# Frank-Wang-oss/GNN_RUL_Benchmarking

Measured on AMD Instinct MI355X. Metric: training samples/sec, C-MAPSS FD004-shaped ST_GCN, higher is better.
Workload: dtype f32 (f16x2-split MFMA operands, fp32 accumulate); 1 GPU; ST_GCN.update (fwd+MSE+bwd+Adam), C-MAPSS FD004-shaped windows [14 sensors x 30], per-GPU batch 65536, dropout 0.2, lr 0.0001, wd 0.0001; per_gpu_batch=65536, global_batch=65536, num_patch=14, patch_size=30, parallelism=dp1, batchnorm=single process, loss_readback=end of run (device-side loss each step)

## Files before the change

### gnn_rul_benchmarking_amd/csrc/stgcn_train_layout.hpp

```cpp
#pragma once
#include "stgcn_device.hpp"
#include "stgcn_host.hpp"

namespace rulgnn {

struct StepScratch {
    uint32_t drop_key[8];
    float lr_over_bc1, inv_sqrt_bc2;
    double bn_count;
    uint32_t pad[4];
};
static_assert(sizeof(StepScratch) == 64, "step scratch layout");
constexpr uint32_t WS_CLEAN_TOKEN = 0x52554C43u;

struct HeadScalars {
    StepScratch* sc;
    uint64_t seed, step;
    int L, has_adam;
    int64_t adam_step;
    float lr, beta1, beta2;
    double bn_count;
};
__device__ __forceinline__ void head_scalars(const HeadScalars& h, int tid) {
    StepScratch* sc = h.sc;
    if (tid == 0) {
        sc->bn_count = h.bn_count;
        if (sc->pad[1] != WS_CLEAN_TOKEN) {
            sc->pad[0] = 2u;
            sc->pad[2] = 0u;
        }
        sc->pad[1] = 0u;
    }
    if (tid >= 64 && tid < 72) sc->drop_key[tid - 64] = tid - 64 < h.L ? dropout_layer_key(h.seed, h.step, tid - 64) : 0u;
    if (h.has_adam && tid == 128) {
        const double bc1 = 1.0 - pow((double)h.beta1, (double)h.adam_step);
        const double bc2 = 1.0 - pow((double)h.beta2, (double)h.adam_step);
        sc->lr_over_bc1 = (float)((double)h.lr / bc1);
        sc->inv_sqrt_bc2 = (float)(1.0 / sqrt(bc2));
    }
}

constexpr int CELL_REPLICAS = 16;
__host__ __device__ constexpr int cell_fwd(int L) { (void)L; return 0; }
__host__ __device__ constexpr int cell_bwd(int L) { return 2 * L * 2 * F; }
__host__ __device__ constexpr int cell_loss(int L) { return 2 * (2 * L * 2 * F); }
__host__ __device__ constexpr int cell_stride(int L) { return 2 * (2 * L * 2 * F) + 8; }
__host__ __device__ __forceinline__ StepScratch* step_scratch(double* cells, int L) {
    return reinterpret_cast<StepScratch*>(cells + CELL_REPLICAS * cell_stride(L));
}
__host__ __device__ __forceinline__ unsigned* step_barrier(double* cells, int L) {
    return reinterpret_cast<unsigned*>(reinterpret_cast<char*>(step_scratch(cells, L)) + sizeof(StepScratch));
}
__device__ __forceinline__ double cell_sum(const double* cells, int L, int i) {
    double v = 0.0;
#pragma unroll
    for (int r = 0; r < CELL_REPLICAS; ++r) v += cells[r * cell_stride(L) + i];
    return v;
}

constexpr int BN_TABLE_ROWS = 7;
template <bool COHERENT = false>
__device__ __forceinline__ void bn_pair_to_lds(const double* cells, const float* prm, float* bnc, int L, int N, bool fwd, int b, int lane) {
    const int CS = cell_stride(L);
    const int base = (fwd ? cell_fwd(L) : cell_bwd(L)) + b * 2 * F;
    double v = 0.0;
    if (lane < 2 * F) {
        if constexpr (COHERENT) {
            double t[CELL_REPLICAS];
#pragma unroll
            for (int r = 0; r < CELL_REPLICAS; ++r) t[r] = __hip_atomic_load(&cells[r * CS + base + lane], __ATOMIC_RELAXED, __HIP_MEMORY_SCOPE_AGENT);
#pragma unroll
            for (int r = 0; r < CELL_REPLICAS; ++r) v += t[r];
        } else {
#pragma unroll
        for (int r = 0; r < CELL_REPLICAS; ++r) v += cells[r * CS + base + lane];
        }
    }
    const double s1 = v, s2 = __shfl(v, (lane + F) & 63, 64);
    if (lane < F) {
        const int c = lane;
        const double cnt = step_scratch(const_cast<double*>(cells), L)->bn_count;
        float* o = bnc + b * BN_TABLE_ROWS * F;
        if (fwd) {
            const double mean = s1 / cnt;
            double var = s2 / cnt - mean * mean;
            var = var < 0.0 ? 0.0 : var;
            const double istd = 1.0 / sqrt(var + (double)BN_EPS);
            const int LS = layer_stride(N);
            const double g = prm[(b / 2) * LS + off_bn_g(N, b % 2) + c];
            o[0 * F + c] = (float)mean;
            o[1 * F + c] = (float)istd;
            o[2 * F + c] = (float)g;
            o[3 * F + c] = prm[(b / 2) * LS + off_bn_b(N, b % 2) + c];
            o[4 * F + c] = (float)(g * istd);
        } else {
            o[5 * F + c] = (float)(s1 / cnt);
            o[6 * F + c] = (float)(s2 / cnt);
        }
    }
}

}
```

### gnn_rul_benchmarking_amd/csrc/stgcn_train_mx.hip

```cpp
#include <algorithm>
#include <cstdlib>
#include <type_traits>

#include "stgcn_host.hpp"
#include "stgcn_mx.hpp"
#include "stgcn_train_layout.hpp"
#include "stgcn_train_mx.hpp"
#include "stgcn_train_mx_ops.hpp"

namespace rulgnn {

#ifdef MXP_TRACE
__device__ unsigned mxp_ts[128];
__device__ int mxp_n;
__device__ unsigned mxp_id[128];
#define MXP_MARKI(ID) do { if (PERSIST && blockIdx.x == 0 && threadIdx.x == 0 && mxp_n < 128) { mxp_id[mxp_n] = ID; mxp_ts[mxp_n++] = (unsigned)wall_clock64(); } } while (0)
#define MXP_MARK() MXP_MARKI(0)
#else
#define MXP_MARK() do {} while (0)
#define MXP_MARKI(ID) do {} while (0)
#endif
template <int L, int KIND, int IDX, int NFIX, bool PERSIST>
__device__ __forceinline__ void mxt_phase_body(const MxTrainK& a, float* smem_all, unsigned target) {
    MXP_MARKI(100 + KIND * 10 + IDX);
    const int N = NFIX ? NFIX : a.N;
    const int LS = layer_stride(N);
    const int lane = threadIdx.x & 63, wave = threadIdx.x >> 6;
    const int g = lane >> 4, col = lane & 15;
    constexpr int NBN = 2 * L;
    constexpr int CS = cell_stride(L);
    constexpr int LY = KIND == PH_TOP ? L - 1 : IDX / 2;
    constexpr int BLK = KIND == PH_TOP ? 1 : IDX % 2;
    constexpr bool WITH_PREV = KIND == PH_F && BLK == 0 && LY >= 1;
    constexpr bool BWD_PREV = KIND == PH_G && BLK == 0 && LY >= 1;
    constexpr int LIN = WITH_PREV ? LY - 1 : LY;
    constexpr bool GRAD_IN = KIND == PH_G && (BLK == 1 || LY >= 1);
    constexpr bool GRAD_TOP = GRAD_IN && LY == L - 1;
    constexpr bool NEED_SB = KIND == PH_G && BLK == 0;
    static_assert(!(KIND == PH_F && IDX == 0), "F_0 is stgcn_train_f0_mx_kernel");

    const int XF = 40 * N;
    constexpr int AF = 220;
    constexpr int SH_BNC = (NBN * MXT_BNC * F + 3) & ~3;
    float* const bnc = smem_all;
    float* const red = smem_all + SH_BNC;
    double* const pairbuf = reinterpret_cast<double*>(red + MXT_RED_FLOATS);
    const int off_zero = 0;
    const int off_scr = off_zero + MXT_ZERO_FLOATS;
    const int off_sh = off_scr + MXT_SCRATCH_FLOATS;
    const int off_X = off_sh + MXT_SHIFT_FLOATS;
    const int off_A = off_X + XF;
    const int off_SB = off_A + AF;
    const int off_DX = off_SB + (NEED_SB ? XF : 0);
    const int off_XP = off_DX + (GRAD_IN ? XF : 0);
    const int wave_floats = off_XP + (BWD_PREV ? XF : 0);
    float* const smem = smem_all + SH_BNC + MXT_RED_FLOATS + 2 * MXT_WAVES * (2 * F + 2) + wave * wave_floats;
    u32x2* const sh_tile = reinterpret_cast<u32x2*>(smem + off_sh);

    int64_t tile = (int64_t)blockIdx.x * MXT_WAVES + wave;
    const int64_t tstride = (int64_t)gridDim.x * MXT_WAVES;

    auto dma = [&](const float* src, int off, int bytes) {
        if constexpr (NFIX != 0) {
            if (bytes == 160 * NFIX) { dma_tile_fixed<160 * NFIX>(src, smem + off, lane); return; }
            if (bytes == 32 * NFIX) { dma_tile_fixed<32 * NFIX>(src, smem + off, lane); return; }
        }
        if (bytes == 4 * AF) { dma_tile_fixed<4 * AF>(src, smem + off, lane); return; }
        dma_tile(src, smem + off, bytes, lane);
    };
    auto req_XA = [&](int64_t t) {
        dma(a.xrec[LIN] + t * XF, off_X, 4 * XF);
        dma(a.arec + t * AF, off_A, 4 * AF);
    };
    auto req_SB = [&](int64_t t) { if constexpr (NEED_SB) dma(a.sb + t * XF, off_SB, 4 * XF); };
    auto req_DX = [&](int64_t t) {
        if constexpr (GRAD_TOP) dma(a.dtop + t * (8 * N), off_DX, 32 * N);
        else if constexpr (GRAD_IN) dma(a.dx + t * XF, off_DX, 4 * XF);
    };
    auto req_XP = [&](int64_t t) { if constexpr (BWD_PREV) dma(a.qrec[LY] + t * XF, off_XP, 4 * XF); };
    if (tile < a.ntiles) { req_XA(tile); req_SB(tile); req_DX(tile); req_XP(tile); }

    for (int i = lane; i < MXT_ZERO_FLOATS; i += 64) smem[off_zero + i] = 0.f;
    if (lane < 2) sh_tile[64 + 65 * lane] = u32x2{0u, 0u};
    constexpr int M0_LY = (KIND == PH_F && BLK == 0) ? 1 : 2;
    constexpr int M1_LY = (KIND == PH_F && BLK == 0) ? 0 : ((KIND == PH_F) ? 1 : ((KIND == PH_G && BLK == 0) ? 0 : 2));
    MXP_MARKI(1);
    LayerRaw rc, rp;
    layer_raw(rc, a.prm, LY, N, g, col, M0_LY, M1_LY);
    if constexpr (WITH_PREV) layer_raw(rp, a.prm, LY - 1, N, g, col, 2, 2);
    ConvOp wT = ConvOp{u32x4{0u, 0u, 0u, 0u}, u32x4{0u, 0u, 0u, 0u}};
    ThetaOp thN = ThetaOp{u32x4{0u, 0u, 0u, 0u}, u32x4{0u, 0u, 0u, 0u}};
    u32x4 ident = u32x4{0u, 0u, 0u, 0u};
    ConvRaw wT_raw = ConvRaw{{0.f, 0.f, 0.f, 0.f}, {0.f, 0.f, 0.f, 0.f}};
    ThetaRaw thN_raw = ThetaRaw{{0.f, 0.f, 0.f, 0.f}};
    if constexpr (KIND == PH_G) {
        wT_raw = conv_bwd_raw(a.prm + LY * LS + off_conv_w(N, BLK), g, col);
        if constexpr (BLK == 0 && LY >= 1) thN_raw = theta_n_raw(a.prm + LY * LS, N, g, col);
        unsigned w[4];
#pragma unroll
        for (int r = 0; r < 4; ++r) w[r] = (4 * g + r == col) ? 0x3C00u : 0u;
        const unsigned p01 = w[0] | (w[1] << 16), p23 = w[2] | (w[3] << 16);
        ident = u32x4{p01, p23, p01, p23};
    }
    {
        constexpr int FW0 = WITH_PREV ? 2 * LY - 2 : 2 * LY;
        constexpr int NFW = (KIND == PH_F && BLK == 1) || (KIND == PH_G && BLK == 0) ? 1 : 2;
        static_assert(NFW + (KIND == PH_G ? 1 : 0) <= MXT_WAVES, "one reduction pair per wavefront");
        MXP_MARKI(2);
        if constexpr (PERSIST) {
            if (threadIdx.x == 0) {
                unsigned* const ctr = step_barrier(a.cells, L);
                unsigned spins = 0;
                while (__hip_atomic_load(ctr, __ATOMIC_RELAXED, __HIP_MEMORY_SCOPE_AGENT) < target) {
                    __builtin_amdgcn_s_sleep(1);
                    if (++spins > (1u << 22)) { atomicOr(&step_scratch(a.cells, L)->pad[0], 4u); break; }
                }
            }
            __syncthreads();
        }
        constexpr bool COH = PERSIST;
        MXP_MARKI(3);
        if (wave < NFW) bn_pair_to_lds<COH>(a.cells, a.prm, bnc, L, N, true, FW0 + wave, lane);
        if (KIND == PH_G && wave == NFW) bn_pair_to_lds<COH>(a.cells, a.prm, bnc, L, N, false, IDX, lane);
        if constexpr (KIND == PH_G) {
            wT = conv_bwd_pack(wT_raw);
            if constexpr (BLK == 0 && LY >= 1) thN = theta_pack(thN_raw);
        }
        __syncthreads();
    }
    MXP_MARKI(4);
    LayerK kc;
    layer_constants(kc, rc, bnc, LY, g, col, M0_LY, M1_LY);
    LayerK kp;
    if constexpr (WITH_PREV) layer_constants(kp, rp, bnc, LY - 1, g, col, 2, 2);
    float bA[3] = {0.f, 0.f, 0.f}, bk1[3] = {0.f, 0.f, 0.f}, bk2[3] = {0.f, 0.f, 0.f};
    if constexpr (KIND == PH_G) {
        const float* q = bnc + IDX * MXT_BNC * F;
#pragma unroll
        for (int r = 0; r < 3; ++r) {
            const int c = slot_chan(4 * g + r);
            bA[r] = c >= 0 ? q[4 * F + c] : 0.f;
            bk1[r] = c >= 0 ? q[5 * F + c] * a.gscale : 0.f;
            bk2[r] = c >= 0 ? q[6 * F + c] * a.gscale : 0.f;
        }
    }
    float fc1w[16], fc1wT[16];
    float fc1b = 0.f, fc2w = 0.f, fc2b = 0.f;
    if constexpr (KIND == PH_TOP) {
        const int colc = col < N ? col : 0;
#pragma unroll
        for (int k = 0; k < 16; ++k) {
            const int kc2 = k < N ? k : 0;
            const float v = a.prm[off_fc1_w(N, L) + colc * N + kc2], vt = a.prm[off_fc1_w(N, L) + kc2 * N + colc];
            fc1w[k] = (col < N && k < N) ? v : 0.f;
            fc1wT[k] = (col < N && k < N) ? vt : 0.f;
        }
        const float b1 = a.prm[off_fc1_b(N, L) + colc], w2 = a.prm[off_fc2_w(N, L) + colc];
        fc1b = col < N ? b1 : 0.f;
        fc2w = col < N ? w2 : 0.f;
        fc2b = a.prm[off_fc2_b(N, L)];
    }

    const bool col_ok = col < N;
    const float colm = col_ok ? 1.f : 0.f;
    const int pitch = 4 * N;
    int xoff[3], aoff[3], chan[3];
#pragma unroll
    for (int r = 0; r < 3; ++r) {
        const int c = slot_chan(4 * g + r);
        chan[r] = c;
        xoff[r] = (c >= 0 && col_ok) ? c * pitch + col : -1;
    }
    {
        const int cc = slot_chan(col);
#pragma unroll
        for (int r = 0; r < 3; ++r) {
            const int c = slot_chan(4 * g + r);
            aoff[r] = (c >= 0 && cc >= 0) ? sym(c, cc) : -1;
        }
    }
    auto ld_tile = [&](int base, float (&v)[4][3]) {
#pragma unroll
        for (int s = 0; s < 4; ++s)
#pragma unroll
            for (int r = 0; r < 3; ++r) v[s][r] = smem[(xoff[r] >= 0 ? base + xoff[r] : off_zero) + s * N];
    };
    auto st_tile = [&](float* dst, const float (&v)[4][3], int ns) {
#pragma unroll
        for (int s = 0; s < 4; ++s)
            if (s < ns) {
#pragma unroll
                for (int r = 0; r < 3; ++r)
                    if (xoff[r] >= 0) dst[xoff[r] + s * N] = v[s][r];
            }
    };
    const int sh_rd1 = col >= 1 ? lane - 1 : 64, sh_rd2 = col >= 2 ? lane - 2 : 64;
    int sh_rd1_lo = sh_rd1 + 65, sh_rd2_lo = sh_rd2 + 65;
    const int sh_bk = col + (BLK == 0 ? 1 : 2) < 16 ? lane + (BLK == 0 ? 1 : 2) : 64;
    int sh_bk_lo = sh_bk + 65;
    asm volatile("" : "+v"(sh_rd1_lo), "+v"(sh_rd2_lo), "+v"(sh_bk_lo));
    const unsigned t_bias = g == 3 ? 0x3C00u << 16 : 0u;
    uint32_t dkey[L];
#pragma unroll
    for (int l = 0; l < L; ++l) dkey[l] = step_scratch(a.cells, L)->drop_key[l];
    uint32_t dro[3];
#pragma unroll
    for (int r = 0; r < 3; ++r) dro[r] = (uint32_t)((chan[r] >= 0 ? chan[r] : 0) * N + col);
    const bool use_drop = a.dropout_p > 0.f;

    float s_a[3] = {0.f, 0.f, 0.f}, s_b[3] = {0.f, 0.f, 0.f};
    f32x4 acc_w0 = {0.f, 0.f, 0.f, 0.f}, acc_w1 = {0.f, 0.f, 0.f, 0.f};
    f32x4 acc_th = {0.f, 0.f, 0.f, 0.f};
    float acc_b = 0.f, acc_w2 = 0.f, acc_b2 = 0.f, acc_loss = 0.f;
    const float inv_gb = 1.0f / (float)a.global_batch;

    auto stage_T = [&](const auto& X, const auto& adjB, auto& T, auto& xo) {
        constexpr int NS = std::extent_v<std::remove_reference_t<decltype(T)>>;
#pragma unroll
        for (int s = 0; s < NS; ++s) {
            const Split2 p01 = split2(X[s][0], X[s][1]), p2 = split2(X[s][2], 0.f);
            const Op2 o = {u32x4{p01.hi, p2.hi, p01.hi, p2.hi}, u32x4{p01.lo, p2.lo, p01.lo, p2.lo}};
            xo[s] = o;
            T[s] = mfma16z(o.h, adjB[s]);
            T[s] = mfma16(o.l, adjB[s], T[s]);
        }
        __builtin_amdgcn_sched_barrier(0);
    };
    auto stage_Hp = [&](const auto& T, const ThetaOp& th, auto& Hp) {
        constexpr int NS = std::extent_v<std::remove_reference_t<decltype(Hp)>>;
#pragma unroll
        for (int s = 0; s < NS; ++s) {
            const Split2 p01 = split2(T[s][0], T[s][1]), p23 = split2(T[s][2], T[s][3]);
            const u32x4 ta = {p01.hi, p23.hi | t_bias, p01.lo, p23.lo};
            Hp[s] = mfma16z(ta, th.hi);
            Hp[s] = mfma16(ta, th.lo, Hp[s]);
        }
        __builtin_amdgcn_sched_barrier(0);
    };
    auto stage_conv = [&](const auto& D, float partner, const ConvOp& w, int rd, int rd_lo, auto& z, auto& keep, auto& keep_sh) {
        constexpr int NS = std::extent_v<std::remove_reference_t<decltype(z)>>;
        u32x4 bh[NS], bl[NS];
#pragma unroll
        for (int s = 0; s < NS; ++s) {
            const Pk p = pack3(D[s][0], D[s][1], D[s][2], partner);
            const Shifted prev = shift_read(sh_tile, rd, rd_lo, lane, p);
            bh[s] = cat(p.hi, prev.hi);
            bl[s] = cat(p.lo, prev.lo);
            keep[s] = p;
            keep_sh[s] = prev;
            __builtin_amdgcn_sched_barrier(0);
        }
        __builtin_amdgcn_sched_barrier(0);
#pragma unroll
        for (int s = 0; s < NS; ++s) {
            z[s] = mfma16z(w.hi, bh[s]);
            z[s] = mfma16(w.hi, bl[s], z[s]);
            z[s] = mfma16(w.lo, bh[s], z[s]);
        }
        __builtin_amdgcn_sched_barrier(0);
    };
    auto leaky_of = [&](const auto& Hp, auto& H) {
        constexpr int NS = std::extent_v<std::remove_reference_t<decltype(H)>>;
#pragma unroll
        for (int s = 0; s < NS; ++s) {
            keep_until_here(Hp[s][3]);
#pragma unroll
            for (int r = 0; r < 3; ++r) H[s][r] = fmaf((1.f - LEAKY) / (1.f + LEAKY), __builtin_fabsf(Hp[s][r]), Hp[s][r]);
        }
    };
    auto layer_full = [&](float (&X)[4][3], const u32x4 (&adjB)[4], const LayerK& k, uint32_t key, const uint32_t (&sbase)[4],
                          float (*xh1_out)[4][3], float (*y2_out)[4][3], float (*q_out)[4][3], uint32_t* mbits_out) {
        f32x4 T[4], Hp[4], z[4];
        float H[4][3], V[4][3];
        Op2 xo[4];
        Pk pk[4];
        Shifted ps[4];
        stage_T(X, adjB, T, xo);
        stage_Hp(T, k.th, Hp);
        leaky_of(Hp, H);
        stage_conv(H, 1.0f, k.w[0], sh_rd1, sh_rd1_lo, z, pk, ps);
#pragma unroll
        for (int s = 0; s < 4; ++s) {
            keep_until_here(z[s][3]);
#pragma unroll
            for (int r = 0; r < 3; ++r) {
                const float y1 = fmaf(k.gam[0][r], z[s][r], k.bet[0][r]);
                V[s][r] = relu2(fmaf(2.f, H[s][r], relu2(y1)));
            }
        }
        stage_conv(V, 1.0f, k.w[1], sh_rd2, sh_rd2_lo, z, pk, ps);
        uint32_t mbits = 0u;
#pragma unroll
        for (int s = 0; s < 4; ++s) {
            keep_until_here(z[s][3]);
#pragma unroll
            for (int r = 0; r < 3; ++r) {
                const float xh = z[s][r];
                const float y2 = fmaf(k.gam[1][r], xh, k.bet[1][r]);
                if (xh1_out) (*xh1_out)[s][r] = xh;
                if (y2_out) (*y2_out)[s][r] = y2;
                float o1 = fmaf(0.5f, relu2(y2), 0.25f * V[s][r]);
                bool keep = true;
                if (use_drop) {
                    const uint32_t h = lowbias32((sbase[s] + dro[r]) ^ key);
                    keep = h >= a.drop_thr;
                    o1 = keep ? o1 * a.drop_scale : 0.f;
                    mbits |= keep ? 1u << (3 * s + r) : 0u;
                }
                if (q_out) (*q_out)[s][r] = (keep && y2 > 0.f) ? xh : INFINITY;
                X[s][r] = fmaf(colm, o1, X[s][r]);
            }
        }
        *mbits_out = mbits;
    };

    bool pend = false;
    int64_t pend_tile = 0;
    int pend_ns = 0;
    float pend_v[4][3], pend_q[4][3];
    float pend_top0 = 0.f, pend_top1 = 0.f, pend_pred = 0.f;
    uint32_t pend_m = 0u;
    uint32_t mask_next = 0u;
    constexpr bool MASK_IN = KIND == PH_G && BLK == 1;
    if constexpr (MASK_IN) {
        if (use_drop && tile < a.ntiles) mask_next = a.mrec[LY][tile * 64 + lane];
    }
#pragma unroll
    for (int s = 0; s < 4; ++s)
#pragma unroll
        for (int r = 0; r < 3; ++r) pend_v[s][r] = pend_q[s][r] = 0.f;

    MXP_MARKI(5);
    for (; tile < a.ntiles; tile += tstride) {
        const int64_t s0 = tile * 4;
        const int ns_tile = (int)((a.B - s0) < 4 ? (a.B - s0) : 4);
        auto tile_body = [&](auto FULL_) {
        constexpr bool FULL = decltype(FULL_)::value;
        const int ns = FULL ? 4 : ns_tile;
        const int64_t nt = tile + tstride;
        asm volatile("s_waitcnt vmcnt(0) lgkmcnt(0)" ::: "memory");
        __builtin_amdgcn_wave_barrier();
        if (pend) {
            if constexpr (WITH_PREV) {
                st_tile(a.xrec[LY] + pend_tile * XF, pend_v, pend_ns);
                st_tile(a.qrec[LY] + pend_tile * XF, pend_q, pend_ns);
                if (use_drop) a.mrec[LY - 1][pend_tile * 64 + lane] = pend_m;
            }
            if constexpr (KIND == PH_G && BLK == 1) st_tile(a.sb + pend_tile * XF, pend_v, pend_ns);
            if constexpr (BWD_PREV) st_tile(a.dx + pend_tile * XF, pend_v, pend_ns);
            if constexpr (KIND == PH_TOP) {
                if (g < pend_ns && col_ok && a.do_backward) {
                    float* p = a.dtop + pend_tile * (8 * N) + g * N + col;
                    p[0] = pend_top0;
                    p[pitch] = pend_top1;
                }
                if (g < pend_ns && col == 0) a.pred[pend_tile * 4 + g] = pend_pred;
                if (use_drop && a.do_backward) a.mrec[LY][pend_tile * 64 + lane] = pend_m;
            }
        }
        float X[4][3];
        u32x4 adjB[4];
        ld_tile(off_X, X);
        {
#pragma unroll
            for (int s = 0; s < 4; ++s) {
                unsigned q[3];
#pragma unroll
                for (int r = 0; r < 3; ++r) q[r] = __builtin_bit_cast(unsigned, smem[(aoff[r] >= 0 ? off_A + aoff[r] : off_zero) + s * 55]);
                adjB[s] = u32x4{__builtin_amdgcn_perm(q[1], q[0], 0x05040100u), q[2] & 0xFFFFu, __builtin_amdgcn_perm(q[1], q[0], 0x07060302u), q[2] >> 16};
            }
            if (ns < 4) {
#pragma unroll
                for (int s = 0; s < 4; ++s)
                    if (s >= ns) { adjB[s] = u32x4{0u, 0u, 0u, 0u}; X[s][0] = X[s][1] = X[s][2] = 0.f; }
            }
        }
        asm volatile("s_waitcnt lgkmcnt(0)" ::: "memory");
        __builtin_amdgcn_wave_barrier();
        if (nt < a.ntiles) req_XA(nt);
        uint32_t sbase[4];
#pragma unroll
        for (int s = 0; s < 4; ++s) sbase[s] = (uint32_t)((a.sample_offset + s0 + s) * F) * (uint32_t)N;
        const bool any_row = true;
        (void)any_row;

        if constexpr (KIND == PH_F) {
            if constexpr (WITH_PREV) {
                layer_full(X, adjB, kp, dkey[LY - 1], sbase, nullptr, nullptr, &pend_q, &pend_m);
#pragma unroll
                for (int s = 0; s < 4; ++s)
#pragma unroll
                    for (int r = 0; r < 3; ++r) pend_v[s][r] = X[s][r];
            }
            f32x4 T[4], Hp[4], z[4];
            float H[4][3];
            Op2 xo[4];
            Pk pk[4];
            Shifted ps[4];
            stage_T(X, adjB, T, xo);
            stage_Hp(T, kc.th, Hp);
            leaky_of(Hp, H);
            if constexpr (BLK == 0) {
                stage_conv(H, 0.f, kc.w[0], sh_rd1, sh_rd1_lo, z, pk, ps);
            } else {
                stage_conv(H, 1.0f, kc.w[0], sh_rd1, sh_rd1_lo, z, pk, ps);
                float V[4][3];
#pragma unroll
                for (int s = 0; s < 4; ++s) {
                    keep_until_here(z[s][3]);
#pragma unroll
                    for (int r = 0; r < 3; ++r) V[s][r] = relu2(fmaf(2.f, H[s][r], relu2(fmaf(kc.gam[0][r], z[s][r], kc.bet[0][r]))));
                }
                stage_conv(V, 0.f, kc.w[1], sh_rd2, sh_rd2_lo, z, pk, ps);
            }
#pragma unroll
            for (int s = 0; s < 4; ++s) {
                keep_until_here(z[s][3]);
                if (s < ns) {
#pragma unroll
                    for (int r = 0; r < 3; ++r) {
                        const float zv = z[s][r] * colm;
                        s_a[r] += zv;
                        s_b[r] = fmaf(zv, zv, s_b[r]);
                    }
// ... 318 lines not shown
            if constexpr (BLK == 1 || LY >= 1) { pend = true; pend_tile = tile; pend_ns = ns; }
        }
        };
        if (ns_tile == 4) tile_body(std::true_type{});
        else tile_body(std::false_type{});
    }

    MXP_MARKI(6);
    if (pend) {
        if constexpr (WITH_PREV) {
            st_tile(a.xrec[LY] + pend_tile * XF, pend_v, pend_ns);
            st_tile(a.qrec[LY] + pend_tile * XF, pend_q, pend_ns);
            if (use_drop) a.mrec[LY - 1][pend_tile * 64 + lane] = pend_m;
        }
        if constexpr (KIND == PH_G && BLK == 1) st_tile(a.sb + pend_tile * XF, pend_v, pend_ns);
        if constexpr (BWD_PREV) st_tile(a.dx + pend_tile * XF, pend_v, pend_ns);
        if constexpr (KIND == PH_TOP) {
            if (g < pend_ns && col_ok && a.do_backward) {
                float* p = a.dtop + pend_tile * (8 * N) + g * N + col;
                p[0] = pend_top0;
                p[pitch] = pend_top1;
            }
            if (g < pend_ns && col == 0) a.pred[pend_tile * 4 + g] = pend_pred;
            if (use_drop && a.do_backward) a.mrec[LY][pend_tile * 64 + lane] = pend_m;
        }
    }

    MXP_MARKI(7);
    StepScratch* const sc = step_scratch(a.cells, L);
    bool bad = false;
    const bool has_pair = (KIND == PH_F) || (KIND == PH_TOP && a.do_backward) || (KIND == PH_G && IDX > 0);
    constexpr int PBW = 2 * F + 2;
    if (has_pair) {
#pragma unroll
        for (int r = 0; r < 3; ++r) {
            double da = (double)s_a[r], db = (double)s_b[r];
#pragma unroll
            for (int off = 8; off >= 1; off >>= 1) {
                da += __shfl_xor(da, off, 16);
                db += __shfl_xor(db, off, 16);
            }
            if (col == 0 && chan[r] >= 0) {
                pairbuf[wave * PBW + chan[r]] = da;
                pairbuf[wave * PBW + F + chan[r]] = db;
            }
        }
    }
    if constexpr (KIND == PH_TOP) {
        float vl = acc_loss;
        vl += __shfl_xor(vl, 16, 64);
        vl += __shfl_xor(vl, 32, 64);
        if (lane == 0) pairbuf[wave * PBW + 2 * F] = (double)vl;
    }
    __syncthreads();
    MXP_MARKI(8);
    if (has_pair && threadIdx.x < 2 * F) {
        double* cell = a.cells + (int64_t)(blockIdx.x % CELL_REPLICAS) * CS;
        if (KIND == PH_F) cell += cell_fwd(L) + IDX * 2 * F;
        else if (KIND == PH_TOP) cell += cell_bwd(L) + (NBN - 1) * 2 * F;
        else cell += cell_bwd(L) + (IDX - 1) * 2 * F;
        double v = 0.0;
#pragma unroll
        for (int w = 0; w < MXT_WAVES; ++w) v += pairbuf[w * PBW + threadIdx.x];
        atomicAdd(cell + threadIdx.x, KIND == PH_F ? v : v * (double)a.inv_gscale);
    }
    if (KIND == PH_TOP && threadIdx.x == 2 * F) {
        double v = 0.0;
#pragma unroll
        for (int w = 0; w < MXT_WAVES; ++w) v += pairbuf[w * PBW + 2 * F];
        atomicAdd(a.cells + (int64_t)(blockIdx.x % CELL_REPLICAS) * CS + cell_loss(L), v);
        bad |= !(v <= 1.0e300 && v >= 0.0);
    }
    if constexpr (KIND == PH_F) return;
    if (KIND == PH_TOP && !a.do_backward) {
        if (__any(bad) && lane == 0) atomicOr(&sc->pad[0], 1u);
        return;
    }

    MXP_MARKI(9);
    const float us = a.inv_gscale;
    const int NN = N * N;
    int rbase = 0, rlen = 0;
    float* const red2 = smem_all + SH_BNC + MXT_RED_FLOATS + 2 * MXT_WAVES * (2 * F + 2);
    for (int w = 0; w < 2; ++w) {
        if ((wave >> 1) == w) {
            float* const img = (wave & 1) ? red2 : red;
            auto put = [&](int idx, float v) { img[idx] = (w == 0) ? v : img[idx] + v; };
            if constexpr (KIND == PH_TOP) {
#pragma unroll
                for (int r = 0; r < 4; ++r) {
                    const int j = 4 * g + r;
                    if (j < N && col_ok) put(j * N + col, acc_th[r]);
                }
                float vb = acc_b, vw = acc_w2, v2 = acc_b2;
                vb += __shfl_xor(vb, 16, 64); vb += __shfl_xor(vb, 32, 64);
                vw += __shfl_xor(vw, 16, 64); vw += __shfl_xor(vw, 32, 64);
                v2 += __shfl_xor(v2, 16, 64); v2 += __shfl_xor(v2, 32, 64);
                if (g == 0 && col_ok) { put(NN + col, vb); put(NN + N + col, vw); }
                if (lane == 0) put(NN + 2 * N, v2);
            }
            if constexpr (KIND == PH_G) {
                const int ci = slot_chan(col);
                const int cbase = BLK == 0 ? NN + N : 0;
                const float ws = BLK == 1 ? 0.25f : 1.f;
#pragma unroll
                for (int r = 0; r < 3; ++r) {
                    const int co = chan[r];
                    if (co >= 0 && ci >= 0) {
                        put(cbase + (co * F + ci) * 2 + 1, acc_w0[r] * ws);
                        put(cbase + (co * F + ci) * 2 + 0, acc_w1[r] * ws);
                    }
                }
                if constexpr (BLK == 0) {
#pragma unroll
                    for (int r = 0; r < 4; ++r) {
                        const int j = 4 * g + r;
                        if (j < N && col_ok) put(j * N + col, acc_th[r]);
                    }
                    float vb = acc_b;
                    vb += __shfl_xor(vb, 16, 64); vb += __shfl_xor(vb, 32, 64);
                    if (g == 0 && col_ok) put(NN + col, vb);
                }
            }
        }
        __syncthreads();
    }
    MXP_MARKI(10);
    if constexpr (KIND == PH_TOP) { rbase = off_fc1_w(N, L); rlen = NN + 2 * N + 1; }
    else if constexpr (BLK == 0) { rbase = LY * LS + off_theta_w(N); rlen = NN + N + CONVW; }
    else { rbase = LY * LS + off_conv_w(N, 1); rlen = CONVW; }
    float* row = a.gpart + (size_t)blockIdx.x * a.pcount + rbase;
    for (int i = threadIdx.x; i < rlen; i += 64 * MXT_WAVES) {
        const float v = (red[i] + red2[i]) * us;
        row[i] = v;
        bad |= !finite_f(v);
    }
    if (__any(bad) && lane == 0) atomicOr(&sc->pad[0], 1u);
}

template <int L, int KIND, int IDX, int NFIX>
__global__ __launch_bounds__(64 * MXT_WAVES, MX_WAVES_PER_SIMD) void stgcn_train_mx_kernel(MxTrainK a) {
    extern __shared__ __attribute__((aligned(16))) float smem_all[];
    mxt_phase_body<L, KIND, IDX, NFIX, false>(a, smem_all, 0u);
}

template <int L, int KIND, int IDX, int NFIX>
__device__ __forceinline__ void mxt_persist_phase(const MxTrainK& a, float* smem_all, unsigned& arrived_phases) {
    mxt_phase_body<L, KIND, IDX, NFIX, true>(a, smem_all, arrived_phases * gridDim.x);
    constexpr bool PERSIST = true;
    MXP_MARKI(11);
    asm volatile("s_waitcnt vmcnt(0) lgkmcnt(0)" ::: "memory");
    MXP_MARKI(12);
    __syncthreads();
    if (threadIdx.x == 0) __hip_atomic_fetch_add(step_barrier(a.cells, L), 1u, __ATOMIC_RELAXED, __HIP_MEMORY_SCOPE_AGENT);
    ++arrived_phases;
}
template <int L, int NFIX, int I>
struct MxtPersistChain {
    static __device__ __forceinline__ void forward(const MxTrainK& a, float* smem_all, unsigned& n) {
        if constexpr (I > 1) MxtPersistChain<L, NFIX, I - 1>::forward(a, smem_all, n);
        mxt_persist_phase<L, PH_F, I, NFIX>(a, smem_all, n);
    }
    static __device__ __forceinline__ void backward(const MxTrainK& a, float* smem_all, unsigned& n) {
        mxt_persist_phase<L, PH_G, I, NFIX>(a, smem_all, n);
        if constexpr (I > 0) MxtPersistChain<L, NFIX, I - 1>::backward(a, smem_all, n);
    }
};
template <int L, int NFIX>
__global__ __launch_bounds__(64 * MXT_WAVES, MX_WAVES_PER_SIMD) void stgcn_train_mx_persist_kernel(MxTrainK a) {
    extern __shared__ __attribute__((aligned(16))) float smem_all[];
    unsigned n = 0;
    MxtPersistChain<L, NFIX, 2 * L - 1>::forward(a, smem_all, n);
    mxt_persist_phase<L, PH_TOP, 0, NFIX>(a, smem_all, n);
    MxtPersistChain<L, NFIX, 2 * L - 1>::backward(a, smem_all, n);
#ifdef MXP_TRACE
    if (blockIdx.x == 0 && threadIdx.x == 0) {
        for (int i = 0; i < mxp_n; ++i) {
            if (mxp_id[i] >= 100) printf("\nphase %u:", mxp_id[i]);
            else printf(" [%u] +%u", mxp_id[i], mxp_ts[i] - mxp_ts[i - 1]);
        }
        printf("\n");
        mxp_n = 0;
    }
#endif
}

static size_t mxt_lds_bytes(int L, int kind, int idx, int N) {
    const int blk = kind == PH_TOP ? 1 : idx % 2, ly = kind == PH_TOP ? L - 1 : idx / 2;
    const bool need_sb = kind == PH_G && blk == 0, grad_in = kind == PH_G && (blk == 1 || ly >= 1), bwd_prev = kind == PH_G && blk == 0 && ly >= 1;
    const int XF = 40 * N;
    const size_t wave = (size_t)MXT_ZERO_FLOATS + MXT_SCRATCH_FLOATS + MXT_SHIFT_FLOATS + XF + 220 + (need_sb ? XF : 0) + (grad_in ? XF : 0) +
                        (bwd_prev ? XF : 0);
    const size_t shared = (size_t)((2 * L * MXT_BNC * F + 3) & ~3) + MXT_RED_FLOATS + 2 * MXT_WAVES * (2 * F + 2);
    return (shared + MXT_WAVES * wave) * sizeof(float);
}

template <int L, int KIND, int IDX, int NFIX>
static int mxt_launch(const MxTrainK& k, hipStream_t stream, int max_grid, int* grid_out) {
    auto kern = &stgcn_train_mx_kernel<L, KIND, IDX, NFIX>;
    const size_t lds = mxt_lds_bytes(L, KIND, IDX, k.N);
    if (lds > 80 * 1024) return RULGNN_EUNSUPPORTED;
    if (lds > 48 * 1024 &&
        hipFuncSetAttribute(reinterpret_cast<const void*>(kern), hipFuncAttributeMaxDynamicSharedMemorySize, (int)lds) != hipSuccess)
        return RULGNN_EHIP;
    int dev = 0, cus = 256, per_cu = 0;
    if (hipGetDevice(&dev) == hipSuccess) {
        int v = 0;
        if (hipDeviceGetAttribute(&v, hipDeviceAttributeMultiprocessorCount, dev) == hipSuccess && v > 0) cus = v;
    }
    if (hipOccupancyMaxActiveBlocksPerMultiprocessor(&per_cu, kern, 64 * MXT_WAVES, lds) != hipSuccess || per_cu < 1) per_cu = 1;
    if (per_cu > MX_WAVES_PER_SIMD) per_cu = MX_WAVES_PER_SIMD;
    if (const char* e = getenv("RULGNN_MXT_BLOCKS_PER_CU")) { const int v = atoi(e); if (v > 0) per_cu = v; }
    int64_t grid = (int64_t)cus * per_cu;
    const int64_t want = (k.ntiles + MXT_WAVES - 1) / MXT_WAVES;
    if (grid > want) grid = want;
    if (grid > max_grid) grid = max_grid;
    if (grid_out) *grid_out = (int)grid;
    (void)hipGetLastError();
    hipLaunchKernelGGL(kern, dim3((unsigned)grid), dim3(64 * MXT_WAVES), lds, stream, k);
    return hipGetLastError() == hipSuccess ? RULGNN_OK : RULGNN_EHIP;
}

template <int L, int KIND, int IDX>
static int mxt_launch_n(const MxTrainK& k, hipStream_t stream, int max_grid, int* grid_out) {
    if (k.N == 14) return mxt_launch<L, KIND, IDX, 14>(k, stream, max_grid, grid_out);
    return mxt_launch<L, KIND, IDX, 0>(k, stream, max_grid, grid_out);
}

template <int L, int I>
struct MxtPhase {
    static int run(int kind, int idx, const MxTrainK& k, hipStream_t st, int mg, int* go) {
        if (idx == I) {
            if (kind == PH_F) {
                if constexpr (I >= 1) return mxt_launch_n<L, PH_F, I>(k, st, mg, go);
                else return RULGNN_EINVAL;
            }
            if (kind == PH_G) return mxt_launch_n<L, PH_G, I>(k, st, mg, go);
        }
        if constexpr (I > 0) return MxtPhase<L, I - 1>::run(kind, idx, k, st, mg, go);
        return RULGNN_EINVAL;
    }
};

bool stgcn_train_mx_shape_ok(const rulgnn_stgcn_shape* s, const float* x) {
    const int N = s->num_patch, P = s->patch_size, L = s->num_layers;
    if (N < 2 || N > 15 || L < 1 || L > MX_MAX_LAYERS || s->mpnn_k != 1) return false;
    if (((int64_t)N * P) % 4 != 0 || (reinterpret_cast<uintptr_t>(x) & 15) != 0) return false;
    return true;
}

float stgcn_train_mx_grad_scale(int64_t global_batch) {
    int e = 0;
    while (((int64_t)1 << e) < global_batch && e < 40) ++e;
    return ldexpf(1.0f, e + 3);
}

static MxTrainK mxt_kernel_args(const MxTrainArgs& m) {
    MxTrainK k;
    k.prm = m.prm; k.y = m.y; k.pred = m.pred; k.cells = m.cells; k.gpart = m.gpart;
    for (int l = 0; l < MX_MAX_LAYERS; ++l) { k.xrec[l] = m.xrec[l]; k.qrec[l] = m.qrec[l]; k.mrec[l] = m.mrec[l]; }
    k.arec = m.arec; k.sb = m.sb; k.dx = m.dx; k.dtop = m.dtop;
    k.B = m.B; k.ntiles = (m.B + 3) / 4; k.global_batch = m.global_batch; k.sample_offset = m.sample_offset;
    k.N = m.N; k.pcount = m.pcount;
    k.dropout_p = m.dropout_p; k.drop_scale = m.drop_scale; k.drop_thr = m.drop_thr;
    k.gscale = stgcn_train_mx_grad_scale(m.global_batch);
    k.inv_gscale = 1.0f / k.gscale;
// ... 60 lines not shown
```

Before: 191.3 million samples/s.

## Hoist BN stat and parameter loads ahead of tile DMA and flatten gradient reduction

Splits the BN-statistics conversion into a load step and a finish step. In the non-persistent kernel, the replica cell loads, the fc-head weights, the dropout keys and the first mask are issued before the tile DMA so their latency overlaps with setup. The weight-gradient reduction drops its two-round loop with two barriers: each of the four waves now writes its own LDS image, and a single barrier is followed by a four-way sum. This costs more LDS for the red2 images (three replicas), which could affect occupancy if the LDS sizing is not updated, and holds more registers across setup. Trace markers are also extended to the non-persistent kernel.

```diff
diff --git a/gnn_rul_benchmarking_amd/csrc/stgcn_train_layout.hpp b/gnn_rul_benchmarking_amd/csrc/stgcn_train_layout.hpp
--- a/gnn_rul_benchmarking_amd/csrc/stgcn_train_layout.hpp
+++ b/gnn_rul_benchmarking_amd/csrc/stgcn_train_layout.hpp
@@ -59,39 +59,52 @@
 }
 
 constexpr int BN_TABLE_ROWS = 7;
+struct BnPairRaw {
+    double t[CELL_REPLICAS];
+    double cnt;
+    float g, b;
+};
 template <bool COHERENT = false>
-__device__ __forceinline__ void bn_pair_to_lds(const double* cells, const float* prm, float* bnc, int L, int N, bool fwd, int b, int lane) {
+__device__ __forceinline__ void bn_pair_load(BnPairRaw& p, const double* cells, const float* prm, int L, int N, bool fwd, int b, int lane) {
     const int CS = cell_stride(L);
     const int base = (fwd ? cell_fwd(L) : cell_bwd(L)) + b * 2 * F;
+    if (lane < 2 * F) {
+#pragma unroll
+        for (int r = 0; r < CELL_REPLICAS; ++r) {
+            if constexpr (COHERENT) p.t[r] = __hip_atomic_load(&cells[r * CS + base + lane], __ATOMIC_RELAXED, __HIP_MEMORY_SCOPE_AGENT);
+            else p.t[r] = cells[r * CS + base + lane];
+        }
+    }
+    if (lane < F) {
+        p.cnt = step_scratch(const_cast<double*>(cells), L)->bn_count;
+        if (fwd) {
+            const int LS = layer_stride(N);
+            p.g = prm[(b / 2) * LS + off_bn_g(N, b % 2) + lane];
+            p.b = prm[(b / 2) * LS + off_bn_b(N, b % 2) + lane];
+        }
+    }
+}
+__device__ __forceinline__ void bn_pair_finish(const BnPairRaw& p, float* bnc, bool fwd, int b, int lane) {
     double v = 0.0;
     if (lane < 2 * F) {
-        if constexpr (COHERENT) {
-            double t[CELL_REPLICAS];
 #pragma unroll
-            for (int r = 0; r < CELL_REPLICAS; ++r) t[r] = __hip_atomic_load(&cells[r * CS + base + lane], __ATOMIC_RELAXED, __HIP_MEMORY_SCOPE_AGENT);
-#pragma unroll
-            for (int r = 0; r < CELL_REPLICAS; ++r) v += t[r];
-        } else {
-#pragma unroll
-        for (int r = 0; r < CELL_REPLICAS; ++r) v += cells[r * CS + base + lane];
-        }
+        for (int r = 0; r < CELL_REPLICAS; ++r) v += p.t[r];
     }
     const double s1 = v, s2 = __shfl(v, (lane + F) & 63, 64);
     if (lane < F) {
         const int c = lane;
-        const double cnt = step_scratch(const_cast<double*>(cells), L)->bn_count;
+        const double cnt = p.cnt;
         float* o = bnc + b * BN_TABLE_ROWS * F;
         if (fwd) {
             const double mean = s1 / cnt;
             double var = s2 / cnt - mean * mean;
             var = var < 0.0 ? 0.0 : var;
             const double istd = 1.0 / sqrt(var + (double)BN_EPS);
-            const int LS = layer_stride(N);
-            const double g = prm[(b / 2) * LS + off_bn_g(N, b % 2) + c];
+            const double g = p.g;
             o[0 * F + c] = (float)mean;
             o[1 * F + c] = (float)istd;
             o[2 * F + c] = (float)g;
-            o[3 * F + c] = prm[(b / 2) * LS + off_bn_b(N, b % 2) + c];
+            o[3 * F + c] = p.b;
             o[4 * F + c] = (float)(g * istd);
         } else {
             o[5 * F + c] = (float)(s1 / cnt);
@@ -99,5 +112,11 @@
         }
     }
 }
+template <bool COHERENT = false>
+__device__ __forceinline__ void bn_pair_to_lds(const double* cells, const float* prm, float* bnc, int L, int N, bool fwd, int b, int lane) {
+    BnPairRaw p;
+    bn_pair_load<COHERENT>(p, cells, prm, L, N, fwd, b, lane);
+    bn_pair_finish(p, bnc, fwd, b, lane);
+}
 
 }
diff --git a/gnn_rul_benchmarking_amd/csrc/stgcn_train_mx.hip b/gnn_rul_benchmarking_amd/csrc/stgcn_train_mx.hip
--- a/gnn_rul_benchmarking_amd/csrc/stgcn_train_mx.hip
+++ b/gnn_rul_benchmarking_amd/csrc/stgcn_train_mx.hip
@@ -14,8 +14,18 @@
 __device__ unsigned mxp_ts[128];
 __device__ int mxp_n;
 __device__ unsigned mxp_id[128];
-#define MXP_MARKI(ID) do { if (PERSIST && blockIdx.x == 0 && threadIdx.x == 0 && mxp_n < 128) { mxp_id[mxp_n] = ID; mxp_ts[mxp_n++] = (unsigned)wall_clock64(); } } while (0)
+#define MXP_MARKI(ID) do { if (blockIdx.x == 0 && threadIdx.x == 0 && mxp_n < 128) { mxp_id[mxp_n] = ID; mxp_ts[mxp_n++] = (unsigned)wall_clock64(); } } while (0)
 #define MXP_MARK() MXP_MARKI(0)
+__device__ __forceinline__ void mxp_dump() {
+    if (blockIdx.x == 0 && threadIdx.x == 0) {
+        for (int i = 0; i < mxp_n; ++i) {
+            if (mxp_id[i] >= 100) printf("\nphase %u:", mxp_id[i]);
+            else printf(" [%u] +%u", mxp_id[i], mxp_ts[i] - mxp_ts[i - 1]);
+        }
+        printf("\n");
+        mxp_n = 0;
+    }
+}
 #else
 #define MXP_MARK() do {} while (0)
 #define MXP_MARKI(ID) do {} while (0)
@@ -78,8 +88,15 @@
         else if constexpr (GRAD_IN) dma(a.dx + t * XF, off_DX, 4 * XF);
     };
     auto req_XP = [&](int64_t t) { if constexpr (BWD_PREV) dma(a.qrec[LY] + t * XF, off_XP, 4 * XF); };
-    if (tile < a.ntiles) { req_XA(tile); req_SB(tile); req_DX(tile); req_XP(tile); }
-
+
+    constexpr int FW0 = WITH_PREV ? 2 * LY - 2 : 2 * LY;
+    constexpr int NFW = (KIND == PH_F && BLK == 1) || (KIND == PH_G && BLK == 0) ? 1 : 2;
+    static_assert(NFW + (KIND == PH_G ? 1 : 0) <= MXT_WAVES, "one reduction pair per wavefront");
+    const bool bn_fwd = wave < NFW, bn_mine = bn_fwd || (KIND == PH_G && wave == NFW);
+    const int bn_b = bn_fwd ? FW0 + wave : IDX;
+    BnPairRaw bnraw;
+    if (!PERSIST && bn_mine) bn_pair_load<false>(bnraw, a.cells, a.prm, L, N, bn_fwd, bn_b, lane);
+    __builtin_amdgcn_sched_barrier(0);
     for (int i = lane; i < MXT_ZERO_FLOATS; i += 64) smem[off_zero + i] = 0.f;
     if (lane < 2) sh_tile[64 + 65 * lane] = u32x2{0u, 0u};
     constexpr int M0_LY = (KIND == PH_F && BLK == 0) ? 1 : 2;
@@ -102,10 +119,34 @@
         const unsigned p01 = w[0] | (w[1] << 16), p23 = w[2] | (w[3] << 16);
         ident = u32x4{p01, p23, p01, p23};
     }
+    float fc1w[16], fc1wT[16];
+    float fc1b = 0.f, fc2w = 0.f, fc2b = 0.f;
+    if constexpr (KIND == PH_TOP) {
+        const int colc = col < N ? col : 0;
+#pragma unroll
+        for (int k = 0; k < 16; ++k) {
+            const int kc2 = k < N ? k : 0;
+            const float v = a.prm[off_fc1_w(N, L) + colc * N + kc2], vt = a.prm[off_fc1_w(N, L) + kc2 * N + colc];
+            fc1w[k] = (col < N && k < N) ? v : 0.f;
+            fc1wT[k] = (col < N && k < N) ? vt : 0.f;
+        }
+        const float b1 = a.prm[off_fc1_b(N, L) + colc], w2 = a.prm[off_fc2_w(N, L) + colc];
+        fc1b = col < N ? b1 : 0.f;
+        fc2w = col < N ? w2 : 0.f;
+        fc2b = a.prm[off_fc2_b(N, L)];
+    }
+    uint32_t dkey[L];
+#pragma unroll
+    for (int l = 0; l < L; ++l) dkey[l] = step_scratch(a.cells, L)->drop_key[l];
+    const bool use_drop = a.dropout_p > 0.f;
+    uint32_t mask_next = 0u;
+    constexpr bool MASK_IN = KIND == PH_G && BLK == 1;
+    if constexpr (MASK_IN) {
+        if (use_drop && tile < a.ntiles) mask_next = a.mrec[LY][tile * 64 + lane];
+    }
+    __builtin_amdgcn_sched_barrier(0);
+    if (tile < a.ntiles) { req_XA(tile); req_SB(tile); req_DX(tile); req_XP(tile); }
     {
-        constexpr int FW0 = WITH_PREV ? 2 * LY - 2 : 2 * LY;
-        constexpr int NFW = (KIND == PH_F && BLK == 1) || (KIND == PH_G && BLK == 0) ? 1 : 2;
-        static_assert(NFW + (KIND == PH_G ? 1 : 0) <= MXT_WAVES, "one reduction pair per wavefront");
         MXP_MARKI(2);
         if constexpr (PERSIST) {
             if (threadIdx.x == 0) {
@@ -120,8 +161,10 @@
         }
         constexpr bool COH = PERSIST;
         MXP_MARKI(3);
-        if (wave < NFW) bn_pair_to_lds<COH>(a.cells, a.prm, bnc, L, N, true, FW0 + wave, lane);
-        if (KIND == PH_G && wave == NFW) bn_pair_to_lds<COH>(a.cells, a.prm, bnc, L, N, false, IDX, lane);
+        if (bn_mine) {
+            if constexpr (PERSIST) bn_pair_load<COH>(bnraw, a.cells, a.prm, L, N, bn_fwd, bn_b, lane);
+            bn_pair_finish(bnraw, bnc, bn_fwd, bn_b, lane);
+        }
         if constexpr (KIND == PH_G) {
             wT = conv_bwd_pack(wT_raw);
             if constexpr (BLK == 0 && LY >= 1) thN = theta_pack(thN_raw);
@@ -144,22 +187,6 @@
             bk2[r] = c >= 0 ? q[6 * F + c] * a.gscale : 0.f;
         }
     }
-    float fc1w[16], fc1wT[16];
-    float fc1b = 0.f, fc2w = 0.f, fc2b = 0.f;
-    if constexpr (KIND == PH_TOP) {
-        const int colc = col < N ? col : 0;
-#pragma unroll
-        for (int k = 0; k < 16; ++k) {
-            const int kc2 = k < N ? k : 0;
-            const float v = a.prm[off_fc1_w(N, L) + colc * N + kc2], vt = a.prm[off_fc1_w(N, L) + kc2 * N + colc];
-            fc1w[k] = (col < N && k < N) ? v : 0.f;
-            fc1wT[k] = (col < N && k < N) ? vt : 0.f;
-        }
-        const float b1 = a.prm[off_fc1_b(N, L) + colc], w2 = a.prm[off_fc2_w(N, L) + colc];
-        fc1b = col < N ? b1 : 0.f;
-        fc2w = col < N ? w2 : 0.f;
-        fc2b = a.prm[off_fc2_b(N, L)];
-    }
 
     const bool col_ok = col < N;
     const float colm = col_ok ? 1.f : 0.f;
@@ -200,13 +227,9 @@
     int sh_bk_lo = sh_bk + 65;
     asm volatile("" : "+v"(sh_rd1_lo), "+v"(sh_rd2_lo), "+v"(sh_bk_lo));
     const unsigned t_bias = g == 3 ? 0x3C00u << 16 : 0u;
-    uint32_t dkey[L];
-#pragma unroll
-    for (int l = 0; l < L; ++l) dkey[l] = step_scratch(a.cells, L)->drop_key[l];
     uint32_t dro[3];
 #pragma unroll
     for (int r = 0; r < 3; ++r) dro[r] = (uint32_t)((chan[r] >= 0 ? chan[r] : 0) * N + col);
-    const bool use_drop = a.dropout_p > 0.f;
 
     float s_a[3] = {0.f, 0.f, 0.f}, s_b[3] = {0.f, 0.f, 0.f};
     f32x4 acc_w0 = {0.f, 0.f, 0.f, 0.f}, acc_w1 = {0.f, 0.f, 0.f, 0.f};
@@ -320,11 +343,6 @@
     float pend_v[4][3], pend_q[4][3];
     float pend_top0 = 0.f, pend_top1 = 0.f, pend_pred = 0.f;
     uint32_t pend_m = 0u;
-    uint32_t mask_next = 0u;
-    constexpr bool MASK_IN = KIND == PH_G && BLK == 1;
-    if constexpr (MASK_IN) {
-        if (use_drop && tile < a.ntiles) mask_next = a.mrec[LY][tile * 64 + lane];
-    }
 #pragma unroll
     for (int s = 0; s < 4; ++s)
 #pragma unroll
@@ -340,6 +358,7 @@
         const int64_t nt = tile + tstride;
         asm volatile("s_waitcnt vmcnt(0) lgkmcnt(0)" ::: "memory");
         __builtin_amdgcn_wave_barrier();
+        if (!pend) MXP_MARKI(13);
         if (pend) {
             if constexpr (WITH_PREV) {
                 st_tile(a.xrec[LY] + pend_tile * XF, pend_v, pend_ns);
@@ -824,56 +843,54 @@
     const int NN = N * N;
     int rbase = 0, rlen = 0;
     float* const red2 = smem_all + SH_BNC + MXT_RED_FLOATS + 2 * MXT_WAVES * (2 * F + 2);
-    for (int w = 0; w < 2; ++w) {
-        if ((wave >> 1) == w) {
-            float* const img = (wave & 1) ? red2 : red;
-            auto put = [&](int idx, float v) { img[idx] = (w == 0) ? v : img[idx] + v; };
-            if constexpr (KIND == PH_TOP) {
+    {
+        float* const img = wave == 0 ? red : red2 + (wave - 1) * MXT_RED_FLOATS;
+        auto put = [&](int idx, float v) { img[idx] = v; };
+        if constexpr (KIND == PH_TOP) {
+#pragma unroll
+            for (int r = 0; r < 4; ++r) {
+                const int j = 4 * g + r;
+                if (j < N && col_ok) put(j * N + col, acc_th[r]);
+            }
+            float vb = acc_b, vw = acc_w2, v2 = acc_b2;
+            vb += __shfl_xor(vb, 16, 64); vb += __shfl_xor(vb, 32, 64);
+            vw += __shfl_xor(vw, 16, 64); vw += __shfl_xor(vw, 32, 64);
+            v2 += __shfl_xor(v2, 16, 64); v2 += __shfl_xor(v2, 32, 64);
+            if (g == 0 && col_ok) { put(NN + col, vb); put(NN + N + col, vw); }
+            if (lane == 0) put(NN + 2 * N, v2);
+        }
+        if constexpr (KIND == PH_G) {
+            const int ci = slot_chan(col);
+            const int cbase = BLK == 0 ? NN + N : 0;
+            const float ws = BLK == 1 ? 0.25f : 1.f;
+#pragma unroll
+            for (int r = 0; r < 3; ++r) {
+                const int co = chan[r];
+                if (co >= 0 && ci >= 0) {
+                    put(cbase + (co * F + ci) * 2 + 1, acc_w0[r] * ws);
+                    put(cbase + (co * F + ci) * 2 + 0, acc_w1[r] * ws);
+                }
+            }
+            if constexpr (BLK == 0) {
 #pragma unroll
                 for (int r = 0; r < 4; ++r) {
                     const int j = 4 * g + r;
                     if (j < N && col_ok) put(j * N + col, acc_th[r]);
                 }
-                float vb = acc_b, vw = acc_w2, v2 = acc_b2;
+                float vb = acc_b;
                 vb += __shfl_xor(vb, 16, 64); vb += __shfl_xor(vb, 32, 64);
-                vw += __shfl_xor(vw, 16, 64); vw += __shfl_xor(vw, 32, 64);
-                v2 += __shfl_xor(v2, 16, 64); v2 += __shfl_xor(v2, 32, 64);
-                if (g == 0 && col_ok) { put(NN + col, vb); put(NN + N + col, vw); }
-                if (lane == 0) put(NN + 2 * N, v2);
-            }
-            if constexpr (KIND == PH_G) {
-                const int ci = slot_chan(col);
-                const int cbase = BLK == 0 ? NN + N : 0;
-                const float ws = BLK == 1 ? 0.25f : 1.f;
-#pragma unroll
-                for (int r = 0; r < 3; ++r) {
-                    const int co = chan[r];
-                    if (co >= 0 && ci >= 0) {
-                        put(cbase + (co * F + ci) * 2 + 1, acc_w0[r] * ws);
-                        put(cbase + (co * F + ci) * 2 + 0, acc_w1[r] * ws);
-                    }
-                }
-                if constexpr (BLK == 0) {
-#pragma unroll
-                    for (int r = 0; r < 4; ++r) {
-                        const int j = 4 * g + r;
-                        if (j < N && col_ok) put(j * N + col, acc_th[r]);
-                    }
-                    float vb = acc_b;
-                    vb += __shfl_xor(vb, 16, 64); vb += __shfl_xor(vb, 32, 64);
-                    if (g == 0 && col_ok) put(NN + col, vb);
-                }
-            }
-        }
-        __syncthreads();
-    }
+                if (g == 0 && col_ok) put(NN + col, vb);
+            }
+        }
+    }
+    __syncthreads();
     MXP_MARKI(10);
     if constexpr (KIND == PH_TOP) { rbase = off_fc1_w(N, L); rlen = NN + 2 * N + 1; }
     else if constexpr (BLK == 0) { rbase = LY * LS + off_theta_w(N); rlen = NN + N + CONVW; }
     else { rbase = LY * LS + off_conv_w(N, 1); rlen = CONVW; }
     float* row = a.gpart + (size_t)blockIdx.x * a.pcount + rbase;
     for (int i = threadIdx.x; i < rlen; i += 64 * MXT_WAVES) {
-        const float v = (red[i] + red2[i]) * us;
+        const float v = ((red[i] + red2[MXT_RED_FLOATS + i]) + (red2[i] + red2[2 * MXT_RED_FLOATS + i])) * us;
         row[i] = v;
         bad |= !finite_f(v);
     }
@@ -884,6 +901,9 @@
 __global__ __launch_bounds__(64 * MXT_WAVES, MX_WAVES_PER_SIMD) void stgcn_train_mx_kernel(MxTrainK a) {
     extern __shared__ __attribute__((aligned(16))) float smem_all[];
     mxt_phase_body<L, KIND, IDX, NFIX, false>(a, smem_all, 0u);
+#ifdef MXP_TRACE
+    mxp_dump();
+#endif
 }
 
 template <int L, int KIND, int IDX, int NFIX>
@@ -916,14 +936,7 @@
     mxt_persist_phase<L, PH_TOP, 0, NFIX>(a, smem_all, n);
     MxtPersistChain<L, NFIX, 2 * L - 1>::backward(a, smem_all, n);
 #ifdef MXP_TRACE
-    if (blockIdx.x == 0 && threadIdx.x == 0) {
-        for (int i = 0; i < mxp_n; ++i) {
-            if (mxp_id[i] >= 100) printf("\nphase %u:", mxp_id[i]);
-            else printf(" [%u] +%u", mxp_id[i], mxp_ts[i] - mxp_ts[i - 1]);
-        }
-        printf("\n");
-        mxp_n = 0;
-    }
+    mxp_dump();
 #endif
 }
 
```

Result: faster. 198.1 million samples/s (median of 6 runs) (+3.6%).
